# HKU-BAL/MegaPath-Nano

Measured on AMD Instinct MI355X. Metric: Gbp/min ONT reads aligned+species-assigned vs RefSeq, 1/2/4/8 MI355X, higher is better.
Workload: dtype int32

## Files before the change

### megapath_nano_amd/csrc/fin_kernels.h

```cpp
#pragma once
#include "ext_kernels.h"

namespace mpn {

struct FinJob { int64_t cig_off, code_off; int32_t n_cigar, read, rid, rev, qs1, rs1, qspan, tspan; };
struct FinOut { int32_t n_cigar, qshift, tshift, blen, mlen, n_ambi, dp_max, pad; };
struct FinParams { int8_t mat[25]; int8_t q, e; };

constexpr uint32_t FIN_SAT = 1u << 31;

template <bool IN_LDS>
__global__ __launch_bounds__(64) void aln_finish_wave_kernel(const FinJob *__restrict__ jobs, const int32_t *__restrict__ list, int n_list,
                                                             uint32_t *__restrict__ CIG, uint32_t *__restrict__ AUX, uint8_t *__restrict__ CODES,
                                                             const uint8_t *__restrict__ reads,
                                                             const int64_t *__restrict__ read_off, const int32_t *__restrict__ read_len,
                                                             RefView rv, FinParams prm, FinOut *__restrict__ out,
                                                             const int64_t *__restrict__ code_offs = nullptr) {
    extern __shared__ __attribute__((aligned(16))) uint8_t fin_lds[];
    __shared__ int32_t sum_l[64][8];
    const int lane = threadIdx.x;
    auto sync = []() { if constexpr (IN_LDS) __builtin_amdgcn_fence(__ATOMIC_ACQ_REL, "workgroup"); else __builtin_amdgcn_fence(__ATOMIC_ACQ_REL, "agent"); __builtin_amdgcn_wave_barrier(); };
    auto excl_scan = [&](int v) { int x = v; for (int d = 1; d < 64; d <<= 1) { const int o = __shfl_up(x, d); if (lane >= d) x += o; } return x - v; };
    for (int li = blockIdx.x; li < n_list; li += gridDim.x) {
        const int jid = list[li];
        const FinJob jb = jobs[jid];
        uint32_t *cg = CIG + jb.cig_off;
        int n = jb.n_cigar;
        uint32_t *c_l, *aux;
        uint8_t *q_l;
        if constexpr (IN_LDS) { c_l = reinterpret_cast<uint32_t *>(fin_lds); aux = c_l + n; q_l = reinterpret_cast<uint8_t *>(aux + n); }
        else { c_l = cg; aux = AUX + jb.cig_off; q_l = CODES + (code_offs ? code_offs[li] : jb.code_off); }
        uint8_t *t_l = q_l + ((jb.qspan + 3) & ~3);
        const int64_t roff = read_off[jb.read];
        const int32_t rlen = read_len[jb.read];
        const int64_t g0 = rv.seq_off[jb.rid] + jb.rs1;
        if constexpr (IN_LDS) {
            for (int i0 = 0; i0 < n; i0 += 512) {
                uint32_t v[8];
#pragma unroll
                for (int u = 0; u < 8; ++u) { const int i = i0 + u * 64 + lane; v[u] = i < n ? cg[i] : 0u; }
#pragma unroll
                for (int u = 0; u < 8; ++u) { const int i = i0 + u * 64 + lane; if (i < n) c_l[i] = v[u]; }
            }
        }
        for (int x0 = 0; x0 < jb.qspan; x0 += 4 * 64 * 4) {
            uint32_t v[4];
#pragma unroll
            for (int u = 0; u < 4; ++u) {
                const int x = x0 + 4 * (u * 64 + lane);
                v[u] = 0x4e4e4e4eu;
                if (x < jb.qspan) {
                    const int64_t a = roff + (jb.rev ? rlen - 1 - (jb.qs1 + x) - 3 : jb.qs1 + x);
                    if (a >= 0) __builtin_memcpy(&v[u], reads + a, 4);
                    else for (int j = 0; j < 4; ++j) if (a + j >= 0) reinterpret_cast<uint8_t *>(&v[u])[j] = reads[a + j];
                    if (jb.rev) v[u] = __builtin_bswap32(v[u]);
                }
            }
#pragma unroll
            for (int u = 0; u < 4; ++u) {
                const int x = x0 + 4 * (u * 64 + lane);
                if (x < jb.qspan) {
                    uint32_t packed = 0;
#pragma unroll
                    for (int j = 0; j < 4; ++j) {
                        const int c = nt4_code((uint8_t)(v[u] >> (8 * j)));
                        packed |= (uint32_t)(jb.rev ? (c < 4 ? 3 - c : 4) : c) << (8 * j);
                    }
                    *reinterpret_cast<uint32_t *>(q_l + x) = packed;
                }
            }
        }
        {
            const int n16 = (jb.tspan + 15) >> 4;
            const int sh = 2 * (int)(g0 & 15);
            const int64_t w0 = g0 >> 4, w_last = (g0 + (jb.tspan > 0 ? jb.tspan - 1 : 0)) >> 4;
            for (int i0 = 0; i0 < n16; i0 += 128) {
                unsigned long long w[2];
#pragma unroll
                for (int u = 0; u < 2; ++u) {
                    const int i = i0 + u * 64 + lane;
                    w[u] = 0;
                    if (i < n16) {
                        const unsigned long long lo = rv.seq2[w0 + i], hi = sh && w0 + i + 1 <= w_last ? rv.seq2[w0 + i + 1] : 0u;
                        w[u] = sh ? (lo >> sh | hi << (32 - sh)) & 0xffffffffULL : lo;
                    }
                }
#pragma unroll
                for (int u = 0; u < 2; ++u) {
                    const int i = i0 + u * 64 + lane;
                    if (i < n16) {
                        const int x = i << 4, m = min(16, jb.tspan - x);
                        for (int b = 0; b < m; ++b) t_l[x + b] = (uint8_t)(w[u] >> (2 * b) & 3);
                    }
                }
            }
            if (rv.n_runs > 0) {
                sync();
                int lo = 0, hi = rv.n_runs;
                while (lo < hi) { const int mid = (lo + hi) >> 1; if (rv.nrun_e[mid] <= g0) lo = mid + 1; else hi = mid; }
                for (; lo < rv.n_runs && rv.nrun_s[lo] < g0 + jb.tspan; ++lo) {
                    const int64_t a = rv.nrun_s[lo] > g0 ? rv.nrun_s[lo] - g0 : 0, b = (rv.nrun_e[lo] < g0 + jb.tspan ? rv.nrun_e[lo] : g0 + jb.tspan) - g0;
                    for (int64_t x = a + lane; x < b; x += 64) t_l[x] = 4;
                }
            }
        }
        sync();
        int qshift = 0, tshift = 0;
        if (n > 1) {
            const int per = (n + 63) / 64, k_lo = min(n, lane * per), k_hi = min(n, k_lo + per);
            int qa = 0, ta = 0;
            for (int k = k_lo; k < k_hi; ++k) { const uint32_t op = c_l[k] & 0xf, len = c_l[k] >> 4; qa += op != 2 ? len : 0; ta += op != 1 ? len : 0; }
            int qoff = excl_scan(qa), toff = excl_scan(ta);
            bool shrink = false, any_sat = false;
            for (int k = k_lo; k < k_hi; ++k) {
                const uint32_t op = c_l[k] & 0xf, len = c_l[k] >> 4;
                uint32_t v = 0;
                if (len == 0 && op != 0) shrink = true;
                if (op == 0) { toff += len; qoff += len; }
                else if (op == 1 || op == 2) {
                    if (k > 0 && k < n - 1 && (c_l[k - 1] & 0xf) == 0 && (c_l[k + 1] & 0xf) == 0) {
                        int l;
                        const int prev_len = c_l[k - 1] >> 4;
                        if (op == 1) { for (l = 0; l < prev_len; ++l) if (q_l[qoff - 1 - l] != q_l[qoff + (int)len - 1 - l]) break; }
                        else { for (l = 0; l < prev_len; ++l) if (t_l[toff - 1 - l] != t_l[toff + (int)len - 1 - l]) break; }
                        v = (uint32_t)l;
                        if (l == prev_len) { v |= FIN_SAT; any_sat = true; }
                    }
                    if (op == 1) qoff += len; else toff += len;
                }
                aux[k] = v;
            }
            sync();
            if (__ballot(any_sat) != 0) {
                if (lane == 0) {
                    int qo = 0, to = 0;
                    for (int k = 0; k < n; ++k) {
                        const uint32_t op = c_l[k] & 0xf, len = c_l[k] >> 4, v = aux[k];
                        if (v & FIN_SAT) {
                            const int grown = (int)(c_l[k - 1] >> 4) + (k >= 2 ? (int)(aux[k - 2] & ~FIN_SAT) : 0);
                            int l = (int)(v & ~FIN_SAT);
                            if (op == 1) { for (; l < grown; ++l) if (q_l[qo - 1 - l] != q_l[qo + (int)len - 1 - l]) break; }
                            else { for (; l < grown; ++l) if (t_l[to - 1 - l] != t_l[to + (int)len - 1 - l]) break; }
                            aux[k] = (uint32_t)l | (l == grown ? FIN_SAT : 0u);
                        }
                        qo += op != 2 ? len : 0; to += op != 1 ? len : 0;
                    }
                }
                sync();
            }
            bool pair = false;
            for (int k = k_lo; k < k_hi; ++k) {
                const uint32_t op = c_l[k] & 0xf;
                if (op == 0) {
                    const uint32_t from_left = k > 0 ? aux[k - 1] & ~FIN_SAT : 0u, to_right = k < n - 1 ? aux[k + 1] & ~FIN_SAT : 0u;
                    const uint32_t seen = (c_l[k] >> 4) + from_left, len = seen - to_right;
                    c_l[k] = len << 4;
                    if (seen == 0 || len == 0) shrink = true;
                } else if (k < n - 2 && op + (c_l[k + 1] & 0xf) == 3) pair = true;
            }
            sync();
            if (__ballot(pair) != 0) {
                int sh2 = 0;
                if (lane == 0) {
                    for (int k = 0; k < n - 2; ++k) {
                        if ((c_l[k] & 0xf) > 0 && (c_l[k] & 0xf) + (c_l[k + 1] & 0xf) == 3) {
                            uint32_t l, sacc[3] = {0, 0, 0};
                            for (l = k; l < (uint32_t)n; ++l) {
                                const uint32_t op = c_l[l] & 0xf;
                                if (op == 1 || op == 2 || c_l[l] >> 4 == 0) sacc[op] += c_l[l] >> 4;
                                else break;
                            }
                            if (sacc[1] > 0 && sacc[2] > 0 && l - k > 2) {
                                c_l[k] = sacc[1] << 4 | 1;
                                c_l[k + 1] = sacc[2] << 4 | 2;
                                for (k += 2; k < (int)l; ++k) c_l[k] &= 0xf;
                                sh2 = 1;
                            }
                            k = l;
                        }
                    }
                }
                if (__builtin_amdgcn_readfirstlane(sh2)) shrink = true;
                sync();
            }
            if (__ballot(shrink) != 0) {
                int n2 = n;
                if (lane == 0) {
                    int32_t l = 0;
                    for (int k = 0; k < n; ++k) if (c_l[k] >> 4 != 0) c_l[l++] = c_l[k];
                    n2 = l;
                    l = 0;
                    for (int k = 0; k < n2; ++k)
                        if (k == n2 - 1 || (c_l[k] & 0xf) != (c_l[k + 1] & 0xf)) c_l[l++] = c_l[k];
                        else c_l[k + 1] += c_l[k] >> 4 << 4;
                    n2 = l;
                }
                n = __builtin_amdgcn_readfirstlane(n2);
                sync();
            }
            if (n > 0 && ((c_l[0] & 0xf) == 1 || (c_l[0] & 0xf) == 2)) {
                const int32_t l = c_l[0] >> 4;
                if ((c_l[0] & 0xf) == 1) qshift = l; else tshift = l;
                sync();
                --n;
                for (int k0 = 0; k0 < n; k0 += 64) {
                    const int k = k0 + lane;
                    const uint32_t v = k < n ? c_l[k + 1] : 0u;
                    sync();
                    if (k < n) c_l[k] = v;
                }
                sync();
            }
        }
        {
            const int per = (n + 63) / 64, k_lo = min(n, lane * per), k_hi = min(n, k_lo + per);
            int qa = 0, ta = 0;
            for (int k = k_lo; k < k_hi; ++k) { const uint32_t op = c_l[k] & 0xf, len = c_l[k] >> 4; qa += op != 2 ? len : 0; ta += op != 1 ? len : 0; }
            int qoff = qshift + excl_scan(qa), toff = tshift + excl_scan(ta);
            int32_t blen = 0, mlen = 0, n_ambi_all = 0;
            const int sc_mch = prm.mat[0], sc_mis = prm.mat[1], sc_amb = prm.mat[4];
            int32_t P = 0, mn = 0, PM = NEG_INF, CM = 0;
            bool first = true;
            auto step = [&](int x) {
                P += x;
                if (first) { mn = P; first = false; } else mn = mn < P ? mn : P;
                PM = PM > P ? PM : P;
                const int c = P - mn;
                CM = CM > c ? CM : c;
            };
            for (int k = k_lo; k < k_hi; ++k) {
                const uint32_t op = c_l[k] & 0xf, len = c_l[k] >> 4;
                if (op == 0) {
                    int n_ambi = 0, n_diff = 0;
                    for (uint32_t l = 0; l < len; ++l) {
                        const int cq = q_l[qoff + (int)l], ct = t_l[toff + (int)l];
                        if (ct > 3 || cq > 3) ++n_ambi;
                        else if (ct != cq) ++n_diff;
                        step(ct > 3 || cq > 3 ? sc_amb : ct == cq ? sc_mch : sc_mis);
                    }
                    blen += len - n_ambi; mlen += len - (n_ambi + n_diff); n_ambi_all += n_ambi;
                    toff += len; qoff += len;
                } else if (op == 1) {
                    int n_ambi = 0;
                    for (uint32_t l = 0; l < len; ++l) if (q_l[qoff + (int)l] > 3) ++n_ambi;
                    blen += len - n_ambi; n_ambi_all += n_ambi;
                    step(-(prm.q + prm.e * (int)len));
                    qoff += len;
                } else if (op == 2) {
                    int n_ambi = 0;
                    for (uint32_t l = 0; l < len; ++l) if (t_l[toff + (int)l] > 3) ++n_ambi;
                    blen += len - n_ambi; n_ambi_all += n_ambi;
                    step(-(prm.q + prm.e * (int)len));
                    toff += len;
                }
            }
            sum_l[lane][0] = first ? 1 : 0; sum_l[lane][1] = P; sum_l[lane][2] = first ? 0 : P - mn; sum_l[lane][3] = PM; sum_l[lane][4] = CM;
            for (int d = 32; d; d >>= 1) { blen += __shfl_xor(blen, d); mlen += __shfl_xor(mlen, d); n_ambi_all += __shfl_xor(n_ambi_all, d); }
            sync();
            if (lane == 0) {
                int32_t s = 0, mx = 0;
                for (int l = 0; l < 64; ++l) {
                    if (sum_l[l][0]) continue;
                    const int32_t D = sum_l[l][1], C = sum_l[l][2], PMl = sum_l[l][3], CMl = sum_l[l][4];
                    const int32_t pk = s + PMl > CMl ? s + PMl : CMl;
                    mx = mx > pk ? mx : pk;
                    s = s + D > C ? s + D : C;
                }
                FinOut o;
                o.n_cigar = n; o.qshift = qshift; o.tshift = tshift; o.blen = blen; o.mlen = mlen; o.n_ambi = n_ambi_all; o.dp_max = mx; o.pad = 0;
                out[jid] = o;
            }
        }
        sync();
        if constexpr (IN_LDS) for (int i = lane; i < n; i += 64) cg[i] = c_l[i];
        sync();
    }
}

}
```

Baseline: 14.86.

## Parallelize serial lane-0 CIGAR fixup passes across the wave and use word loads

Replaces the lane-0 serial loops for saturated indel left-shift extension, adjacent I/D pair merging, and zero-length/duplicate-op compaction with wave-parallel versions built on per-lane ranges, ballots and prefix scans. Adds a word-at-a-time backward matcher and 4-byte packed loads in the match-scoring loop for the global-memory (non-LDS) path. The aim is to remove the single-lane serial bottlenecks and the byte-wise global loads in the finishing kernel. This adds complexity, and the chained saturation logic (the FIN_WAS flag) and the parallel compaction must reproduce the serial semantics exactly.

New measurement: 14.74. About the same (-0.8%).

```diff
diff --git a/megapath_nano_amd/csrc/fin_kernels.h b/megapath_nano_amd/csrc/fin_kernels.h
--- a/megapath_nano_amd/csrc/fin_kernels.h
+++ b/megapath_nano_amd/csrc/fin_kernels.h
@@ -8,6 +8,22 @@
 struct FinParams { int8_t mat[25]; int8_t q, e; };
 
 constexpr uint32_t FIN_SAT = 1u << 31;
+constexpr uint32_t FIN_WAS = 1u << 30;
+constexpr uint32_t FIN_LEN = ~(FIN_SAT | FIN_WAS);
+
+template <bool WORDS>
+__device__ __forceinline__ int fin_match_back(const uint8_t *seq, int a, int b, int l, int lim) {
+    if constexpr (WORDS) {
+        for (; l + 4 <= lim; l += 4) {
+            uint32_t x, y;
+            __builtin_memcpy(&x, seq + a - 4 - l, 4);
+            __builtin_memcpy(&y, seq + b - 4 - l, 4);
+            if (x != y) return l + (__builtin_clz(x ^ y) >> 3);
+        }
+    }
+    for (; l < lim; ++l) if (seq[a - 1 - l] != seq[b - 1 - l]) break;
+    return l;
+}
 
 template <bool IN_LDS>
 __global__ __launch_bounds__(64) void aln_finish_wave_kernel(const FinJob *__restrict__ jobs, const int32_t *__restrict__ list, int n_list,
@@ -110,7 +126,8 @@
             const int per = (n + 63) / 64, k_lo = min(n, lane * per), k_hi = min(n, k_lo + per);
             int qa = 0, ta = 0;
             for (int k = k_lo; k < k_hi; ++k) { const uint32_t op = c_l[k] & 0xf, len = c_l[k] >> 4; qa += op != 2 ? len : 0; ta += op != 1 ? len : 0; }
-            int qoff = excl_scan(qa), toff = excl_scan(ta);
+            const int qoff0 = excl_scan(qa), toff0 = excl_scan(ta);
+            int qoff = qoff0, toff = toff0;
             bool shrink = false, any_sat = false;
             for (int k = k_lo; k < k_hi; ++k) {
                 const uint32_t op = c_l[k] & 0xf, len = c_l[k] >> 4;
@@ -119,12 +136,11 @@
                 if (op == 0) { toff += len; qoff += len; }
                 else if (op == 1 || op == 2) {
                     if (k > 0 && k < n - 1 && (c_l[k - 1] & 0xf) == 0 && (c_l[k + 1] & 0xf) == 0) {
-                        int l;
                         const int prev_len = c_l[k - 1] >> 4;
-                        if (op == 1) { for (l = 0; l < prev_len; ++l) if (q_l[qoff - 1 - l] != q_l[qoff + (int)len - 1 - l]) break; }
-                        else { for (l = 0; l < prev_len; ++l) if (t_l[toff - 1 - l] != t_l[toff + (int)len - 1 - l]) break; }
+                        const int l = op == 1 ? fin_match_back<!IN_LDS>(q_l, qoff, qoff + (int)len, 0, prev_len)
+                                              : fin_match_back<!IN_LDS>(t_l, toff, toff + (int)len, 0, prev_len);
                         v = (uint32_t)l;
-                        if (l == prev_len) { v |= FIN_SAT; any_sat = true; }
+                        if (l == prev_len) { v |= FIN_SAT | FIN_WAS; any_sat = true; }
                     }
                     if (op == 1) qoff += len; else toff += len;
                 }
@@ -132,19 +148,23 @@
             }
             sync();
             if (__ballot(any_sat) != 0) {
-                if (lane == 0) {
-                    int qo = 0, to = 0;
-                    for (int k = 0; k < n; ++k) {
-                        const uint32_t op = c_l[k] & 0xf, len = c_l[k] >> 4, v = aux[k];
-                        if (v & FIN_SAT) {
-                            const int grown = (int)(c_l[k - 1] >> 4) + (k >= 2 ? (int)(aux[k - 2] & ~FIN_SAT) : 0);
-                            int l = (int)(v & ~FIN_SAT);
-                            if (op == 1) { for (; l < grown; ++l) if (q_l[qo - 1 - l] != q_l[qo + (int)len - 1 - l]) break; }
-                            else { for (; l < grown; ++l) if (t_l[to - 1 - l] != t_l[to + (int)len - 1 - l]) break; }
-                            aux[k] = (uint32_t)l | (l == grown ? FIN_SAT : 0u);
+                int qo = qoff0, to = toff0;
+                for (int k = k_lo; k < k_hi; ++k) {
+                    const uint32_t op = c_l[k] & 0xf, len = c_l[k] >> 4;
+                    if ((aux[k] & FIN_WAS) && !(k >= 2 && (aux[k - 2] & FIN_WAS))) {
+                        int q2 = qo, t2 = to;
+                        for (int j = k; j < n - 1 && (aux[j] & FIN_WAS); j += 2) {
+                            const uint32_t opj = c_l[j] & 0xf, lenj = c_l[j] >> 4;
+                            const int grown = (int)(c_l[j - 1] >> 4) + (j >= 2 ? (int)(aux[j - 2] & FIN_LEN) : 0);
+                            const int l0 = (int)(aux[j] & FIN_LEN);
+                            const int l = opj == 1 ? fin_match_back<!IN_LDS>(q_l, q2, q2 + (int)lenj, l0, grown)
+                                                   : fin_match_back<!IN_LDS>(t_l, t2, t2 + (int)lenj, l0, grown);
+                            aux[j] = (uint32_t)l | (l == grown ? FIN_SAT : 0u) | FIN_WAS;
+                            const int m = (int)(c_l[j + 1] >> 4);
+                            q2 += (opj != 2 ? (int)lenj : 0) + m; t2 += (opj != 1 ? (int)lenj : 0) + m;
                         }
-                        qo += op != 2 ? len : 0; to += op != 1 ? len : 0;
-                    }
+                    }
+                    qo += op != 2 ? len : 0; to += op != 1 ? len : 0;
                 }
                 sync();
             }
@@ -152,7 +172,7 @@
             for (int k = k_lo; k < k_hi; ++k) {
                 const uint32_t op = c_l[k] & 0xf;
                 if (op == 0) {
-                    const uint32_t from_left = k > 0 ? aux[k - 1] & ~FIN_SAT : 0u, to_right = k < n - 1 ? aux[k + 1] & ~FIN_SAT : 0u;
+                    const uint32_t from_left = k > 0 ? aux[k - 1] & FIN_LEN : 0u, to_right = k < n - 1 ? aux[k + 1] & FIN_LEN : 0u;
                     const uint32_t seen = (c_l[k] >> 4) + from_left, len = seen - to_right;
                     c_l[k] = len << 4;
                     if (seen == 0 || len == 0) shrink = true;
@@ -160,42 +180,69 @@
             }
             sync();
             if (__ballot(pair) != 0) {
-                int sh2 = 0;
-                if (lane == 0) {
-                    for (int k = 0; k < n - 2; ++k) {
-                        if ((c_l[k] & 0xf) > 0 && (c_l[k] & 0xf) + (c_l[k + 1] & 0xf) == 3) {
-                            uint32_t l, sacc[3] = {0, 0, 0};
-                            for (l = k; l < (uint32_t)n; ++l) {
-                                const uint32_t op = c_l[l] & 0xf;
-                                if (op == 1 || op == 2 || c_l[l] >> 4 == 0) sacc[op] += c_l[l] >> 4;
-                                else break;
-                            }
-                            if (sacc[1] > 0 && sacc[2] > 0 && l - k > 2) {
-                                c_l[k] = sacc[1] << 4 | 1;
-                                c_l[k + 1] = sacc[2] << 4 | 2;
-                                for (k += 2; k < (int)l; ++k) c_l[k] &= 0xf;
-                                sh2 = 1;
-                            }
-                            k = l;
+                auto in_run = [&](int k) { const uint32_t c = c_l[k]; return (c & 0xf) != 0 || c >> 4 == 0; };
+                bool merged = false;
+                for (int k = k_lo; k < k_hi; ++k) {
+                    if (!in_run(k) || (k > 0 && in_run(k - 1))) continue;
+                    int j = k;
+                    bool cand = false;
+                    for (; j < n - 2 && in_run(j); ++j) {
+                        const uint32_t o = c_l[j] & 0xf;
+                        if (o > 0 && o + (c_l[j + 1] & 0xf) == 3) { cand = true; break; }
+                    }
+                    if (!cand) continue;
+                    int l;
+                    uint32_t s1 = 0, s2 = 0;
+                    for (l = j; l < n; ++l) {
+                        const uint32_t op = c_l[l] & 0xf, len = c_l[l] >> 4;
+                        if (op == 1) s1 += len; else if (op == 2) s2 += len; else if (len != 0) break;
+                    }
+                    if (s1 > 0 && s2 > 0 && l - j > 2) {
+                        c_l[j] = s1 << 4 | 1;
+                        c_l[j + 1] = s2 << 4 | 2;
+                        for (int m = j + 2; m < l; ++m) c_l[m] &= 0xf;
+                        merged = true;
+                    }
+                }
+                if (__ballot(merged) != 0) shrink = true;
+                sync();
+            }
+            if (__ballot(shrink) != 0) {
+                int base = 0, ctype = -1;
+                uint32_t clen = 0;
+                for (int k0 = 0; k0 < n; k0 += 64) {
+                    const int k = k0 + lane;
+                    const uint32_t v = k < n ? c_l[k] : 0u;
+                    const uint32_t len = v >> 4;
+                    const int op = (int)(v & 0xf);
+                    const unsigned long long m1 = __ballot(len != 0 && op == 1), m2 = __ballot(len != 0 && op == 2), mz = __ballot(len != 0);
+                    const unsigned long long below = mz & ((1ull << lane) - 1);
+                    int pt = ctype;
+                    if (below) { const int p = 63 - __builtin_clzll(below); pt = (m1 >> p & 1) ? 1 : (m2 >> p & 1) ? 2 : 0; }
+                    const bool head = len != 0 && op != pt;
+                    const unsigned long long H = __ballot(head);
+                    uint32_t incl = len;
+                    for (int d = 1; d < 64; d <<= 1) { const uint32_t o = (uint32_t)__shfl_up((int)incl, d); if (lane >= d) incl += o; }
+                    const uint32_t E = incl - len, total = (uint32_t)__shfl((int)incl, 63);
+                    sync();
+                    if (H != 0) {
+                        const int h0 = __builtin_ctzll(H), hl = 63 - __builtin_clzll(H);
+                        if (ctype >= 0) {
+                            const uint32_t e0 = (uint32_t)__shfl((int)E, h0);
+                            if (lane == 0) c_l[base] = (clen + e0) << 4 | (uint32_t)ctype;
+                            ++base;
                         }
-                    }
-                }
-                if (__builtin_amdgcn_readfirstlane(sh2)) shrink = true;
-                sync();
-            }
-            if (__ballot(shrink) != 0) {
-                int n2 = n;
-                if (lane == 0) {
-                    int32_t l = 0;
-                    for (int k = 0; k < n; ++k) if (c_l[k] >> 4 != 0) c_l[l++] = c_l[k];
-                    n2 = l;
-                    l = 0;
-                    for (int k = 0; k < n2; ++k)
-                        if (k == n2 - 1 || (c_l[k] & 0xf) != (c_l[k + 1] & 0xf)) c_l[l++] = c_l[k];
-                        else c_l[k + 1] += c_l[k] >> 4 << 4;
-                    n2 = l;
-                }
-                n = __builtin_amdgcn_readfirstlane(n2);
+                        const unsigned long long above = lane < 63 ? H & ~((2ull << lane) - 1) : 0ull;
+                        const int nx = above ? __builtin_ctzll(above) : 64;
+                        const uint32_t en = (uint32_t)__shfl((int)E, nx & 63);
+                        if (head && nx < 64) c_l[base + __builtin_popcountll(H & ((1ull << lane) - 1))] = (en - E) << 4 | (uint32_t)op;
+                        base += __builtin_popcountll(H) - 1;
+                        ctype = __shfl(op, hl);
+                        clen = total - (uint32_t)__shfl((int)E, hl);
+                    } else clen += total;
+                }
+                if (ctype >= 0) { if (lane == 0) c_l[base] = clen << 4 | (uint32_t)ctype; ++base; }
+                n = base;
                 sync();
             }
             if (n > 0 && ((c_l[0] & 0xf) == 1 || (c_l[0] & 0xf) == 2)) {
@@ -232,8 +279,17 @@
                 const uint32_t op = c_l[k] & 0xf, len = c_l[k] >> 4;
                 if (op == 0) {
                     int n_ambi = 0, n_diff = 0;
+                    uint32_t wq = 0, wt = 0;
                     for (uint32_t l = 0; l < len; ++l) {
-                        const int cq = q_l[qoff + (int)l], ct = t_l[toff + (int)l];
+                        int cq, ct;
+                        if constexpr (IN_LDS) { cq = q_l[qoff + (int)l]; ct = t_l[toff + (int)l]; }
+                        else {
+                            if ((l & 3) == 0) {
+                                if (l + 4 <= len) { __builtin_memcpy(&wq, q_l + qoff + (int)l, 4); __builtin_memcpy(&wt, t_l + toff + (int)l, 4); }
+                                else { wq = wt = 0; for (uint32_t b = 0; l + b < len; ++b) { wq |= (uint32_t)q_l[qoff + (int)(l + b)] << (8 * b); wt |= (uint32_t)t_l[toff + (int)(l + b)] << (8 * b); } }
+                            }
+                            cq = (int)(wq & 0xff); ct = (int)(wt & 0xff); wq >>= 8; wt >>= 8;
+                        }
                         if (ct > 3 || cq > 3) ++n_ambi;
                         else if (ct != cq) ++n_diff;
                         step(ct > 3 || cq > 3 ? sc_amb : ct == cq ? sc_mch : sc_mis);
```
